# LLNL/graph-embed

Hardware: AMD Instinct MI355X
Metric: ForceAtlas iterations/sec + edges/sec, 3-D embed, 10M-vtx R-MAT @1/2/4/8 GPU (higher is better)
Workload: dtype f64

## Files before the change

graph-embed_amd/csrc/ge_sym.hpp:

```cpp
#pragma once

#include <hip/hip_runtime.h>

#include "ge_pair.hpp"
#include "ge_rows.hpp"

namespace ge {

constexpr int kSymT = 256;

template <int D>
struct SymW {
  static constexpr int v = (D + 1 <= 4) ? 4 : 8;
};

__device__ __forceinline__ double agent_ld(const double* p) {
  return __hip_atomic_load(p, __ATOMIC_RELAXED, __HIP_MEMORY_SCOPE_AGENT);
}
__device__ __forceinline__ void agent_st(double* p, double v) {
  __hip_atomic_store(p, v, __ATOMIC_RELAXED, __HIP_MEMORY_SCOPE_AGENT);
}

__device__ __forceinline__ long long rt_now() { return (long long)__builtin_amdgcn_s_memrealtime(); }

constexpr int kColSlots = 128;
constexpr int kSymRing = 128;
constexpr int kRecSlots = 192;
constexpr int kColBase = 64;

__device__ __forceinline__ void step_barrier() { asm volatile("" ::: "memory"); }

template <int D, bool SHARED, bool REPEL_ONE, bool DIAG>
__device__ __forceinline__ void col_step(int sg, int lane, int coff, const double* rec, double* col,
                                         const double (&xr)[D], double dr, double repel,
                                         double (&racc)[D]) {
  const int q = sg - lane;
  const int p = q & (kSymRing - 1);
  const int pc = coff + q;
  double xq[D + 1], c[D];
#pragma unroll
  for (int k = 0; k <= D; ++k) xq[k] = rec[k * kRecSlots + p];
#pragma unroll
  for (int k = 0; k < D; ++k) c[k] = col[k * kColSlots + pc];
  if (DIAG && q == lane) {
#pragma unroll
    for (int k = 0; k < D; ++k) racc[k] = c[k];
  }
  double t[D];
  rep_term<D, SHARED, REPEL_ONE>(xr, xq, dr, xq[D], repel, t);
  if (!SHARED && DIAG && q == lane) {
#pragma unroll
    for (int k = 0; k < D; ++k) t[k] = 0.0;
  }
#pragma unroll
  for (int k = 0; k < D; ++k) {
    racc[k] = racc[k] + t[k];
    col[k * kColSlots + pc] = c[k] - t[k];
  }
  step_barrier();
}

template <int D, bool REPEL_ONE, bool DIAG>
__device__ __forceinline__ void col_steps(bool fast, int s0, int s1, int lane, int coff,
                                          const double* rec, double* col, const double (&xr)[D],
                                          double dr, double repel, double (&racc)[D]) {
  if (fast)
    for (int sg = s0; sg < s1; ++sg)
      col_step<D, true, REPEL_ONE, DIAG>(sg, lane, coff, rec, col, xr, dr, repel, racc);
  else
    for (int sg = s0; sg < s1; ++sg)
      col_step<D, false, REPEL_ONE, DIAG>(sg, lane, coff, rec, col, xr, dr, repel, racc);
}

template <int D, bool REPEL_ONE, bool STAMP>
__device__ __forceinline__ void tile_steps(int tt, int lane, const double* rec, double* col,
                                           const double (&xr)[D], double dr, double repel,
                                           double (&racc)[D], int& fixes) {
  const double* rb = rec + ((64 * tt - lane) & (kSymRing - 1));
  double* cb = col + kColBase - lane;
  int o2 = 2 * kRecSlots;
  asm volatile("" : "+v"(o2));
  const double* rb2 = rb + o2;
  for (int j0 = 0; j0 < 64; j0 += 8) {
    const double* rj = rb + j0;
    const double* rj2 = rb2 + j0;
    double* cj = cb + j0;
#pragma unroll
    for (int jj = 0; jj < 8; ++jj) {
      double* cp = cj + jj;
      double c[D], xq[D + 1];
#pragma unroll
      for (int k = 0; k <= D; ++k)
        xq[k] = (D >= 3 && k >= 2) ? rj2[(k - 2) * kRecSlots + jj] : rj[k * kRecSlots + jj];
#pragma unroll
      for (int k = 0; k < D; ++k) c[k] = cp[k * kColSlots];
      double t[D];
      bool fixed = false;
      rep_term<D, true, REPEL_ONE, true>(xr, xq, dr, xq[D], repel, t, &fixed);
      if (STAMP) fixes += fixed;
#pragma unroll
      for (int k = 0; k < D; ++k) {
        racc[k] = racc[k] + t[k];
        cp[k * kColSlots] = c[k] - t[k];
      }
      step_barrier();
#pragma unroll
      for (int k = 0; k < D; ++k) asm volatile("" : "+v"(racc[k]));
    }
  }
}

template <int D>
__device__ __forceinline__ double* hand_at(double* H, size_t hs, size_t c, int k) {
  return H + k * hs + c;
}

template <int D>
__device__ __forceinline__ void sym_handover(int t, int lane, int done, int ncols, size_t cbase,
                                             const double* col, int at, double* H, size_t hs,
                                             int* tprog) {
  wave_lds_sync();
  const int qo = 64 * t + lane;
  if (qo < ncols) {
    const double* o = col + at + lane;
#pragma unroll
    for (int k = 0; k < D; ++k) agent_st(hand_at<D>(H, hs, cbase + qo, k), o[k * kColSlots]);
  }
  __atomic_signal_fence(__ATOMIC_SEQ_CST);
  __builtin_amdgcn_s_waitcnt(0);
  __atomic_signal_fence(__ATOMIC_SEQ_CST);
  if (lane == 0) __hip_atomic_store(tprog + t, done, __ATOMIC_RELAXED, __HIP_MEMORY_SCOPE_AGENT);
}

__device__ __forceinline__ int seen(const int* flag) {
  return __builtin_amdgcn_readfirstlane(
      __hip_atomic_load(flag, __ATOMIC_RELAXED, __HIP_MEMORY_SCOPE_AGENT));
}

__device__ __forceinline__ void report_give_up(bool give_up, int lane, int* err) {
  if (give_up && lane == 0) __hip_atomic_store(err, 1, __ATOMIC_RELAXED, __HIP_MEMORY_SCOPE_SYSTEM);
}

constexpr int kLook = 16;

template <bool STAMP>
__device__ __forceinline__ long long handover_wait(const int* flag, const int* look, int A,
                                                   int* err, long long limit, bool& give_up,
                                                   bool& spun, bool& lead) {
  spun = lead = false;
  if (give_up) return 0;
  const int f0 = __hip_atomic_load(flag, __ATOMIC_RELAXED, __HIP_MEMORY_SCOPE_AGENT);
  const int l0 = __hip_atomic_load(look, __ATOMIC_RELAXED, __HIP_MEMORY_SCOPE_AGENT);
  lead = __builtin_amdgcn_readfirstlane(l0) >= A;
  if (__builtin_amdgcn_readfirstlane(f0) >= A) return 0;
  spun = true;
  __builtin_amdgcn_s_setprio(0);
  const long long t0 = rt_now();
  for (int k = 1;; ++k) {
    __builtin_amdgcn_s_sleep(1);
    if (seen(flag) >= A) break;
    if ((k & 255) == 0 &&
        (rt_now() - t0 > limit ||
         __builtin_amdgcn_readfirstlane(
             __hip_atomic_load(err, __ATOMIC_RELAXED, __HIP_MEMORY_SCOPE_SYSTEM)))) {
      give_up = true;
      break;
    }
  }
  return STAMP ? rt_now() - t0 : 0;
}

__device__ __forceinline__ void rows_prio(int rem, int quantum) {
  const int lv = quantum > 0 ? rem / quantum : 3;
  if (lv >= 3) __builtin_amdgcn_s_setprio(3);
  else if (lv == 2) __builtin_amdgcn_s_setprio(2);
  else if (lv == 1) __builtin_amdgcn_s_setprio(1);
  else __builtin_amdgcn_s_setprio(0);
}

__device__ __forceinline__ bool sweep_prio(bool spun, bool lead) {
  if (spun) __builtin_amdgcn_s_setprio(0);
  else if (lead) __builtin_amdgcn_s_setprio(2);
  else __builtin_amdgcn_s_setprio(1);
  return !spun;
}

template <int D, bool REPEL_ONE>
__device__ __forceinline__ void rows_block(int lane, int base, int s, int A, const double* X,
                                           const double* DP, double repel, bool repel_ok,
                                           double* tile, double* F, int quantum) {
  constexpr int WV = SymW<D>::v;
  const size_t rb = (size_t)base + 64 * (size_t)A;
  const bool rv = 64 * A + lane < s;
  double xi[D], acc[D], di = 1.0;
#pragma unroll
  for (int k = 0; k < D; ++k) {
    xi[k] = rv ? X[(rb + lane) * D + k] : 0.0;
    acc[k] = 0.0;
  }
  if (rv) di = DP[rb + lane];
  const bool rows_ok = repel_ok && __all(!rv || vertex_ok<D>(xi, di));
  for (int j0 = 0; j0 < s; j0 += 64) {
    const int cnt = min(64, s - j0);
    rows_prio((s - j0) >> 6, quantum);
    wave_lds_sync();
    bool ok = true;
    if (lane < cnt) {
      const size_t c = (size_t)base + j0 + lane;
#pragma unroll
      for (int k = 0; k < D; ++k) tile[lane * WV + k] = X[c * D + k];
      tile[lane * WV + D] = DP[c];
      ok = vertex_ok<D>(&tile[lane * WV], tile[lane * WV + D]);
    }
    wave_lds_sync();
    if (rows_ok && __all(ok)) {
      int jj = 0;
      for (; jj + 1 < cnt; jj += 2) {
        double t0[D], t1[D];
        rep_term<D, true, REPEL_ONE>(xi, &tile[jj * WV], di, tile[jj * WV + D], repel, t0);
        rep_term<D, true, REPEL_ONE>(xi, &tile[(jj + 1) * WV], di, tile[(jj + 1) * WV + D], repel,
                                     t1);
#pragma unroll
        for (int k = 0; k < D; ++k) acc[k] = (acc[k] + t0[k]) + t1[k];
      }
      if (jj < cnt)
        rep_pair<D, true, REPEL_ONE>(xi, &tile[jj * WV], di, tile[jj * WV + D], repel, acc);
    } else {
      for (int jj = 0; jj < cnt; ++jj)
        rep_pair_fb<D, REPEL_ONE>(xi, &tile[jj * WV], di, tile[jj * WV + D], repel,
                                  j0 + jj == 64 * A + lane, acc);
    }
  }
  wave_lds_sync();
  __builtin_amdgcn_s_setprio(0);
  if (rv) {
#pragma unroll
    for (int k = 0; k < D; ++k) F[(rb + lane) * D + k] = acc[k];
  }
}

constexpr int kStampWords = 8;

template <int D, bool REPEL_ONE, bool STAMP>
__device__ __forceinline__ void sweep_unit(int lane, int A, int base, int s, int* tprog,
                                           int (&hint)[3],
                                           const double* __restrict__ X,
                                           const double* __restrict__ DP, double repel,
                                           bool repel_ok, double* __restrict__ F,
                                           double* __restrict__ H, size_t hs, int* err,
                                           long long limit, bool& give_up, double* rec,
                                           double* col, long long& spin, long long& t_first,
                                           double (&rout)[D]) {
  const size_t cbase = (size_t)base + 64 * (size_t)A;
  const bool rv = 64 * A + lane < s;
  double xr[D], racc[D], dr = 0.0;
#pragma unroll
  for (int k = 0; k < D; ++k) {
    xr[k] = rv ? X[(cbase + lane) * D + k] : 0.0;
    racc[k] = 0.0;
  }
  if (rv) dr = DP[cbase + lane];
  const bool rows_ok = repel_ok && __all(!rv || vertex_ok<D>(xr, dr));
  const int ncols = s - 64 * A;
  const int ntiles = (ncols + 63) >> 6;
  bool ok_prev = true;
  for (int tt = 0; tt < ntiles; ++tt) {
    bool spun = false, lead = true;
    if (A > 0) {
      const long long w =
          handover_wait<STAMP>(tprog + tt, tprog + min(tt + kLook, ntiles - 1), A, err, limit,
                               give_up, spun, lead);
      if (STAMP) {
        spin += w;
        hint[1] += spun;
        if (tt == 0) t_first = rt_now();
      }
      __atomic_signal_fence(__ATOMIC_SEQ_CST);
    }
    const int qc = 64 * tt + lane;
    const bool cv = qc < ncols;
    double xc[D], ic[D], dc = 0.0;
#pragma unroll
    for (int k = 0; k < D; ++k) {
      xc[k] = cv ? X[(cbase + qc) * D + k] : 0.0;
      ic[k] = (cv && A > 0) ? agent_ld(hand_at<D>(H, hs, cbase + qc, k)) : 0.0;
    }
    if (cv) dc = DP[cbase + qc];
    const bool ok_cur = __all(!cv || vertex_ok<D>(xc, dc));
    const int p = qc & (kSymRing - 1);
    if (tt > 0) {
#pragma unroll
      for (int k = 0; k < D; ++k) col[k * kColSlots + lane] = col[k * kColSlots + kColBase + lane];
    }
    const int cb = kColBase;
#pragma unroll
    for (int k = 0; k < D; ++k) {
      rec[k * kRecSlots + p] = xc[k];
      col[k * kColSlots + cb + lane] = ic[k];
    }
    rec[D * kRecSlots + p] = dc;
    if (!(tt & 1)) {
#pragma unroll
      for (int k = 0; k < D; ++k) rec[k * kRecSlots + p + kSymRing] = xc[k];
      rec[D * kRecSlots + p + kSymRing] = dc;
    }
    wave_lds_sync();
    const bool raised = sweep_prio(spun, lead);
    if (STAMP) hint[0] += raised;
    const bool fast = rows_ok && ok_cur && ok_prev;
    const int coff = cb - 64 * tt;
    if (tt < 2)
      col_steps<D, REPEL_ONE, true>(fast, 64 * tt, 64 * tt + 64, lane, coff, rec, col, xr, dr,
                                    repel, racc);
    else if (fast)
      tile_steps<D, REPEL_ONE, STAMP>(tt, lane, rec, col, xr, dr, repel, racc, hint[2]);
    else
      col_steps<D, REPEL_ONE, false>(false, 64 * tt, 64 * tt + 64, lane, coff, rec, col, xr, dr,
                                     repel, racc);
    ok_prev = ok_cur;
    if (tt >= 2) sym_handover<D>(tt - 1, lane, A + 1, ncols, cbase, col, cb - 64, H, hs, tprog);
    wave_lds_sync();
  }
  {
    const int p = (64 * ntiles + lane) & (kSymRing - 1);
#pragma unroll
    for (int k = 0; k <= D; ++k) {
      rec[k * kRecSlots + p] = 0.0;
      if (!(ntiles & 1)) rec[k * kRecSlots + p + kSymRing] = 0.0;
    }
#pragma unroll
    for (int k = 0; k < D; ++k) col[k * kColSlots + lane] = col[k * kColSlots + kColBase + lane];
    wave_lds_sync();
  }
  const int s0 = 64 * ntiles, s1 = ncols + 63;
  const int cbd = kColBase, coff = cbd - 64 * ntiles;
  if (ntiles < 2)
    col_steps<D, REPEL_ONE, true>(rows_ok && ok_prev, s0, s1, lane, coff, rec, col, xr, dr, repel,
                                  racc);
  else
    col_steps<D, REPEL_ONE, false>(rows_ok && ok_prev, s0, s1, lane, coff, rec, col, xr, dr, repel,
                                   racc);
  if (ntiles >= 2)
    sym_handover<D>(ntiles - 1, lane, A + 1, ncols, cbase, col, cbd - 64, H, hs, tprog);
  __builtin_amdgcn_s_setprio(0);
#pragma unroll
  for (int k = 0; k < D; ++k) rout[k] = racc[k];
}

__device__ __forceinline__ void stamp_unit(long long* stamps, int qi, long long t_take,
                                           long long t_first, long long spin,
                                           const int (&hint)[3]) {
  long long* w = stamps + (size_t)qi * kStampWords;
  w[0] = t_take;
  w[1] = t_first;
  w[2] = rt_now();
  w[3] = spin;
  w[4] = __builtin_amdgcn_s_getreg((31 << 11) | 4);
  w[5] = __builtin_amdgcn_s_getreg((31 << 11) | 20) | ((long long)hint[2] << 32);
  w[6] = hint[0];
  w[7] = hint[1];
}

constexpr int kUnitSweep = 0, kUnitRows = 1;

template <int D, bool REPEL_ONE, bool STAMP = false>
__global__ void __launch_bounds__(kSymT, 4)
faml_sym_repulse(int nunits, const int4* __restrict__ units, int* __restrict__ queue,
                 const int* __restrict__ pt_ip, const double* __restrict__ X,
                 const double* __restrict__ DP, double repel, double* __restrict__ F,
                 double* __restrict__ H, size_t hs, int* __restrict__ prog,
                 int* __restrict__ err, long long limit, long long* __restrict__ stamps) {
  constexpr int NW = kSymT / 64;
  static_assert(kRecSlots * (D + 1) >= 64 * SymW<D>::v, "row-block tile fits the record ring");
  __shared__ __attribute__((aligned(16))) double srec[NW][kRecSlots * (D + 1)];
  __shared__ __attribute__((aligned(16))) double scol[NW][kColSlots * D];
  const int lane = threadIdx.x & 63;
  double* rec = srec[threadIdx.x >> 6];
  double* col = scol[threadIdx.x >> 6];
  const bool repel_ok = REPEL_ONE || weight_ok(repel);
  bool give_up = false;
  for (;;) {
    int qi = 0;
    if (lane == 0) qi = atomicAdd(queue, 1);
    qi = __builtin_amdgcn_readfirstlane(qi);
    if (qi >= nunits) break;
    long long t_take = 0, t_first = 0, spin = 0;
    int hint[3] = {0, 0, 0};
    if (STAMP) t_take = t_first = rt_now();
    const int4 u = units[qi];
    const int A = u.y;
    const int base = pt_ip[u.x];
    const int s = pt_ip[u.x + 1] - base;
    const size_t rb = (size_t)base + 64 * (size_t)A;
    if (u.w == kUnitRows) {
      rows_block<D, REPEL_ONE>(lane, base, s, A, X, DP, repel, repel_ok, rec, F, u.z);
    } else {
      double racc[D];
      sweep_unit<D, REPEL_ONE, STAMP>(lane, A, base, s, prog + u.z + A, hint, X,
                                      DP, repel, repel_ok, F, H, hs, err, limit, give_up, rec,
                                      col, spin, t_first, racc);
      if (64 * A + lane < s) {
#pragma unroll
        for (int k = 0; k < D; ++k) F[(rb + lane) * D + k] = racc[k];
      }
    }
    if (STAMP && lane == 0) stamp_unit(stamps, qi, t_take, t_first, spin, hint);
    wave_lds_sync();
  }
  report_give_up(give_up, lane, err);
}

}
```

Measured before the change: 8.744.

## Interleave LDS record pairs for 128-bit reads and prefetch next record in tile loop

Changes the LDS record layout from one plane per component to interleaved pairs of doubles, so each record is fetched with vector-of-two loads instead of scalar LDS reads. For D<=3 it also adds a one-step lookahead in the fast tile loop, reading the next slot's record while the current pairwise term is computed, to hide LDS latency. The interleaved layout can change bank-conflict behaviour, and the lookahead holds extra registers that may reduce occupancy.

```diff
diff --git a/graph-embed_amd/csrc/ge_sym.hpp b/graph-embed_amd/csrc/ge_sym.hpp
--- a/graph-embed_amd/csrc/ge_sym.hpp
+++ b/graph-embed_amd/csrc/ge_sym.hpp
@@ -27,6 +27,52 @@
 constexpr int kSymRing = 128;
 constexpr int kRecSlots = 192;
 constexpr int kColBase = 64;
+
+typedef double rec_half __attribute__((ext_vector_type(2)));
+
+#ifndef GE_SYM_HALVES4
+#define GE_SYM_HALVES4 0
+#endif
+
+template <int D>
+struct SymRec {
+  static constexpr int halves = D == 4 ? GE_SYM_HALVES4 : (D + 1) / 2;
+  static constexpr int half_len = 2 * kRecSlots;
+  static constexpr int tail = halves * half_len;
+};
+
+template <int D>
+__device__ __forceinline__ void rec_read(const double* rec, int slot, double (&xq)[D + 1]) {
+  using R = SymRec<D>;
+#pragma unroll
+  for (int h = 0; h < R::halves; ++h) {
+    const rec_half v = *reinterpret_cast<const rec_half*>(rec + h * R::half_len + 2 * slot);
+    xq[2 * h] = v.x;
+    xq[2 * h + 1] = v.y;
+  }
+#pragma unroll
+  for (int k = 2 * R::halves; k <= D; ++k)
+    xq[k] = rec[R::tail + (k - 2 * R::halves) * kRecSlots + slot];
+}
+
+template <int D>
+__device__ __forceinline__ void rec_write(double* rec, int slot, const double (&x)[D], double d) {
+  using R = SymRec<D>;
+  double r[D + 1];
+#pragma unroll
+  for (int k = 0; k < D; ++k) r[k] = x[k];
+  r[D] = d;
+#pragma unroll
+  for (int h = 0; h < R::halves; ++h) {
+    rec_half v;
+    v.x = r[2 * h];
+    v.y = r[2 * h + 1];
+    *reinterpret_cast<rec_half*>(rec + h * R::half_len + 2 * slot) = v;
+  }
+#pragma unroll
+  for (int k = 2 * R::halves; k <= D; ++k)
+    rec[R::tail + (k - 2 * R::halves) * kRecSlots + slot] = r[k];
+}
 
 __device__ __forceinline__ void step_barrier() { asm volatile("" ::: "memory"); }
 
@@ -38,8 +84,7 @@
   const int p = q & (kSymRing - 1);
   const int pc = coff + q;
   double xq[D + 1], c[D];
-#pragma unroll
-  for (int k = 0; k <= D; ++k) xq[k] = rec[k * kRecSlots + p];
+  rec_read<D>(rec, p, xq);
 #pragma unroll
   for (int k = 0; k < D; ++k) c[k] = col[k * kColSlots + pc];
   if (DIAG && q == lane) {
@@ -72,28 +117,39 @@
       col_step<D, false, REPEL_ONE, DIAG>(sg, lane, coff, rec, col, xr, dr, repel, racc);
 }
 
-template <int D, bool REPEL_ONE, bool STAMP>
+template <int D>
+struct SymAhead {
+#ifdef GE_SYM_AHEAD
+  static constexpr bool v = GE_SYM_AHEAD != 0 && D <= 3;
+#else
+  static constexpr bool v = D <= 3;
+#endif
+};
+
+template <int D, bool REPEL_ONE, bool STAMP, bool AHEAD>
 __device__ __forceinline__ void tile_steps(int tt, int lane, const double* rec, double* col,
                                            const double (&xr)[D], double dr, double repel,
                                            double (&racc)[D], int& fixes) {
-  const double* rb = rec + ((64 * tt - lane) & (kSymRing - 1));
+  const int pb = (64 * tt - lane) & (kSymRing - 1);
   double* cb = col + kColBase - lane;
-  int o2 = 2 * kRecSlots;
-  asm volatile("" : "+v"(o2));
-  const double* rb2 = rb + o2;
+  double xn[D + 1];
+  if (AHEAD) rec_read<D>(rec, pb, xn);
   for (int j0 = 0; j0 < 64; j0 += 8) {
-    const double* rj = rb + j0;
-    const double* rj2 = rb2 + j0;
+    const int pj = pb + j0;
     double* cj = cb + j0;
 #pragma unroll
     for (int jj = 0; jj < 8; ++jj) {
       double* cp = cj + jj;
       double c[D], xq[D + 1];
-#pragma unroll
-      for (int k = 0; k <= D; ++k)
-        xq[k] = (D >= 3 && k >= 2) ? rj2[(k - 2) * kRecSlots + jj] : rj[k * kRecSlots + jj];
+      if (AHEAD) {
+#pragma unroll
+        for (int k = 0; k <= D; ++k) xq[k] = xn[k];
+      } else {
+        rec_read<D>(rec, pj + jj, xq);
+      }
 #pragma unroll
       for (int k = 0; k < D; ++k) c[k] = cp[k * kColSlots];
+      if (AHEAD) rec_read<D>(rec, pj + jj + 1, xn);
       double t[D];
       bool fixed = false;
       rep_term<D, true, REPEL_ONE, true>(xr, xq, dr, xq[D], repel, t, &fixed);
@@ -294,16 +350,10 @@
     }
     const int cb = kColBase;
 #pragma unroll
-    for (int k = 0; k < D; ++k) {
-      rec[k * kRecSlots + p] = xc[k];
+    for (int k = 0; k < D; ++k)
       col[k * kColSlots + cb + lane] = ic[k];
-    }
-    rec[D * kRecSlots + p] = dc;
-    if (!(tt & 1)) {
-#pragma unroll
-      for (int k = 0; k < D; ++k) rec[k * kRecSlots + p + kSymRing] = xc[k];
-      rec[D * kRecSlots + p + kSymRing] = dc;
-    }
+    rec_write<D>(rec, p, xc, dc);
+    if (!(tt & 1)) rec_write<D>(rec, p + kSymRing, xc, dc);
     wave_lds_sync();
     const bool raised = sweep_prio(spun, lead);
     if (STAMP) hint[0] += raised;
@@ -313,7 +363,8 @@
       col_steps<D, REPEL_ONE, true>(fast, 64 * tt, 64 * tt + 64, lane, coff, rec, col, xr, dr,
                                     repel, racc);
     else if (fast)
-      tile_steps<D, REPEL_ONE, STAMP>(tt, lane, rec, col, xr, dr, repel, racc, hint[2]);
+      tile_steps<D, REPEL_ONE, STAMP, SymAhead<D>::v>(tt, lane, rec, col, xr, dr, repel, racc,
+                                                      hint[2]);
     else
       col_steps<D, REPEL_ONE, false>(false, 64 * tt, 64 * tt + 64, lane, coff, rec, col, xr, dr,
                                      repel, racc);
@@ -323,11 +374,11 @@
   }
   {
     const int p = (64 * ntiles + lane) & (kSymRing - 1);
-#pragma unroll
-    for (int k = 0; k <= D; ++k) {
-      rec[k * kRecSlots + p] = 0.0;
-      if (!(ntiles & 1)) rec[k * kRecSlots + p + kSymRing] = 0.0;
-    }
+    double zero[D];
+#pragma unroll
+    for (int k = 0; k < D; ++k) zero[k] = 0.0;
+    rec_write<D>(rec, p, zero, 0.0);
+    if (!(ntiles & 1)) rec_write<D>(rec, p + kSymRing, zero, 0.0);
 #pragma unroll
     for (int k = 0; k < D; ++k) col[k * kColSlots + lane] = col[k * kColSlots + kColBase + lane];
     wave_lds_sync();
```

New measurement: 8.917, median of 6. 2.0% higher.
